# Sachin-A/TraceWeaver

Measured on AMD Instinct MI355X. Metric: spans/sec reconstructed + assignment accuracy vs ground truth, higher is better.
Workload: dtype int64 timestamps, f64 scores; 1 GPU; media_microservices shape (6 services, E in {1,1,1,1,2,4}), 100000 requests/service x 16 replicas per GPU, concurrency 1.6, two-pass reconstruction, device mixture refit; spans_per_gpu=25600000, spans_total=25600000, parallelism=units sharded, 1 rank(s), backend none

## Files before the change

traceweaver_amd/csrc/tw_engine.hip:

```cpp
#include <algorithm>
#include <chrono>
#include <cmath>
#include <cstdio>
#include <cstdlib>
#include <cstring>
#include <functional>
#include <string>
#include <type_traits>
#include <utility>
#include <vector>

#include <hip/hip_runtime.h>
#include <rocprim/rocprim.hpp>

#include "traceweaver_amd.h"
#include "tw_kernels.h"
#include "tw_fit.h"
#include "tw_eval.h"
#include "tw_skip.h"
#include "tw_load.h"
#include "tw_baselines.h"
#include "tw_stitch.h"
#include "tw_attr.h"
#include "tw_conf.h"
// ... 24 lines not shown
struct Knobs {
    int tile;
    int tile_threads;
    int tile_single;
    int tile_single_threads;
    int tile_pair;
    int tile_pair_threads;
    int tile_rank;
    int block_params;
    int coop;
    int set_hw_queues;
    int pipeline;
    int sig_hash_bits;
    int debug_lists;
    int stage_min_tiles;
    int tile_sub;
    int lean_pool;
    int split_twins, defer_min_e, lean_min_e, lean_grid, tile_max_deep;
    int64_t part_slots_max;
    int part_budget_deep;
    int fit_sort;
    int stage_gate;
    int fit_spec;
    int fit_order;
};

Knobs read_knobs() {
    Knobs K;
    K.tile = std::min(std::max(env_int("TW_TILE", kTile), 1), kTile);
    K.tile_threads = std::min(std::max(env_int("TW_TILE_THREADS", 2), 1), 4);
    K.tile_single = env_int("TW_TILE_SINGLE", 1);
    K.tile_single_threads = std::min(std::max(env_int("TW_TILE_SINGLE_THREADS", 1), 1), 4);
    K.tile_pair = env_int("TW_TILE_PAIR", 1);
    K.tile_pair_threads = std::min(std::max(env_int("TW_TILE_PAIR_THREADS", 2), 1), 2);
    K.tile_rank = env_int("TW_TILE_RANK", 1) != 0 ? 1 : 0;
    K.block_params = env_int("TW_BLOCK_PARAMS", 1);
    K.coop = std::min(std::max(env_int("TW_COOP_THREADS", kCoop), 1), kCoop);
    K.set_hw_queues = env_int("TW_SET_HW_QUEUES", 0);
    K.pipeline = env_int("TW_CLASS_PIPELINE", 1);
    K.sig_hash_bits = std::min(std::max(env_int("TW_SIG_HASH_BITS", 64), 1), 64);
    K.debug_lists = env_int("TW_DEBUG_LISTS", 0);
    K.stage_min_tiles = env_int("TW_STAGE_MIN_TILES", 1024);
    K.tile_sub = std::max(env_int("TW_TILE_SUB", 8), 1);
    K.lean_pool = std::min(std::max(env_int("TW_LEAN_POOL", 512), 1), 4096);
    K.split_twins = env_int("TW_SPLIT_TWINS", 2);
    K.defer_min_e = env_int("TW_DEFER_MIN_E", 5);
    K.lean_min_e = env_int("TW_LEAN_MIN_E", 5);
    K.lean_grid = std::max(env_int("TW_LEAN_GRID", TW_LEAN_GRID), 1);
    K.tile_max_deep = std::min(std::max(env_int("TW_TILE_MAX_DEEP", kTileMax), 0), kTileMax);
    K.part_slots_max = (int64_t)std::max(env_int("TW_PART_SLOTS_MAX", 16 << 20), 1024);
    K.part_budget_deep = env_int("TW_PART_BUDGET_DEEP", 2);
    K.fit_sort = env_int("TW_FIT_SORT", 0);
    K.stage_gate = env_int("TW_STAGE_GATE", 1);
    K.fit_spec = env_int("TW_FIT_SPEC", 1) != 0 ? 1 : 0;
    K.fit_order = env_int("TW_FIT_ORDER", 1) != 0 ? 1 : 0;
    return K;
}

struct Mt19937 {
    uint32_t mt[624];
    int idx = 624;
    explicit Mt19937(uint32_t seed = 0u) {
        mt[0] = seed;
        for (int i = 1; i < 624; i++) mt[i] = 1812433253u * (mt[i - 1] ^ (mt[i - 1] >> 30)) + (uint32_t)i;
    }
    uint32_t next() {
        if (idx >= 624) {
            for (int i = 0; i < 624; i++) {
                const uint32_t y = (mt[i] & 0x80000000u) | (mt[(i + 1) % 624] & 0x7fffffffu);
                mt[i] = mt[(i + 397) % 624] ^ (y >> 1) ^ ((y & 1u) ? 0x9908b0dfu : 0u);
            }
            idx = 0;
        }
        uint32_t y = mt[idx++];
        y ^= y >> 11;
        y ^= (y << 7) & 0x9d2c5680u;
        y ^= (y << 15) & 0xefc60000u;
        y ^= y >> 18;
// ... 40 lines not shown
    void* sort_tmp = nullptr;
    size_t sort_tmp_bytes = 0;
    double* mix_p_dev = nullptr;
    int32_t* mix_n_dev = nullptr;
    double* mix_c_dev = nullptr;
    double* gaps_sorted = nullptr;
    double* fit_models = nullptr;
    double* fit_uval = nullptr;
    int32_t *fit_ustart = nullptr, *fit_row_n = nullptr, *fit_row_uniq = nullptr;
    double* fit_centres = nullptr;
    hipEvent_t fit_fork = nullptr, fit_join = nullptr;
    double *fit_spec_centres = nullptr, *fit_spec_p = nullptr;
    int32_t *fit_spec_failed = nullptr, *fit_spec_ctr = nullptr;
    int32_t fit_spec_count[2] = {0, 0};
    double *fit_tape = nullptr, *fit_tape100 = nullptr;
    int64_t* fit_tape_off = nullptr;
    int64_t fit_tape_cap = 0;
    bool fit_runs_pending = false;
    bool fit_prepared = false;
    int32_t hard_pass1[kMaxEp + 1] = {};
    int8_t wide_pass1[kMaxEp + 1] = {};
    int32_t split_pass1[kMaxEp + 1] = {};
    bool pass1_done = false;
    std::vector<int32_t> fit_rows_h;
    bool fit_rows_h_valid = false;
    std::vector<int32_t> fit_order_h;
    int32_t* fit_order_dev = nullptr;
    double fit_order_host_ms = 0.0;
    Mt19937 fit_rng;
    uint32_t fit_seed = 0;
    int32_t* slot_unit = nullptr;
    int32_t* tile_ids = nullptr;
    int32_t* ctr = nullptr;
    int64_t ctr_round_ints = 0, ctr_pass_ints = 0;
    int32_t tile_cls_off[kMaxEp + 2] = {};
    BlockRef* blk_tab = nullptr;
    int32_t blk_cls_off[kMaxEp + 2] = {};
    uint32_t *seg_gap = nullptr, *seg_gap_end = nullptr, *seg_gap_dst = nullptr;
    unsigned long long *comp_a = nullptr, *comp_b = nullptr;
    int64_t comp_cap = 0, n_gap_scored = 0;
    int32_t *truth = nullptr, *in_trace = nullptr;
    uint8_t* trace_bad = nullptr;
    unsigned long long* eval_counts = nullptr;
    int64_t n_traces = 0, trace_cap = 0;
    uint8_t* slot_scored = nullptr;
    int64_t n_gap_rows = 0;
    unsigned long long* key_acc = nullptr;
    double fit_ms = 0.0;
    int rounds = 0;
    bool skip_mode = false;
// ... 226 lines not shown
        if (side.values) (void)hipFree(side.values);
        if (side.off) (void)hipFree(side.off);
        if (side.count) (void)hipFree(side.count);
        if (side.sum) (void)hipFree(side.sum);
        side = tw_engine::HistSide{};
    }
    void* rest[] = {e->hist_tile_off, e->hist_inv, e->hist_counters, e->hist_src_off, e->hist_src_values, e->hist_src_count, e->hist_src_sum};
    for (void* q : rest)
        if (q) (void)hipFree(q);
    e->hist_tile_off = nullptr; e->hist_inv = nullptr; e->hist_counters = nullptr; e->hist_plan_cap = 0; e->hist_inv_cap = 0;
    e->hist_src_off = e->hist_src_values = nullptr; e->hist_src_count = e->hist_src_sum = nullptr; e->hist_src_seg_cap = 0; e->hist_src_cap = 0;
    e->hist_cur = 0; e->hist_C = 0; e->hist_G = 0; e->hist_items = 0; e->hist_pushes = 0;
}

void chist_free(tw_engine* e) {
    ChistDev& H = e->CH;
    void* all[] = {H.table, H.off, H.entries, H.hash, H.stamp, H.cls, H.cell, H.src_hash, H.src_id, H.new_src, H.chunk_sum, H.counters, e->ch_up};
    for (void* q : all)
        if (q) (void)hipFree(q);
    H = ChistDev{};
    e->ch_mode = 0; e->ch_G = 0; e->ch_pushes = 0; e->ch_src_cap = 0; e->ch_up = nullptr; e->ch_up_bytes = 0;
}

void free_all(tw_engine* e) {
    for (void* q : e->allocs) (void)hipFree(q);
    e->allocs.clear();
    e->orig_is = e->orig_ie = e->orig_os = e->orig_oe = nullptr; e->orig_truth = e->orig_trace = nullptr;
    e->truth = nullptr; e->in_trace = nullptr; e->trace_bad = nullptr; e->eval_counts = nullptr; e->n_traces = 0; e->trace_cap = 0;
    drop_buffers(e);
    e->state = ST_EMPTY;
}

const char* kernel_error_text(int code) {
    switch (code) {
        case TW_ERR_WINDOW_WIDTH: return "an incoming span has more candidate spans at one endpoint than the candidate bitmap holds";
        case TW_ERR_WINDOW_SIZE: return "a window holds more than TW_MAX_WINDOW incoming spans";
        case TW_ERR_NAN_PARAMS: return "a parameter block holds a single sample (std = NaN); the reference aborts here (n_in % 100 == 1)";
        case TW_ERR_SKIP_PARAMS: return "skip mode: the scorer needs a (mean, std) pair that BuildDistributions did not produce (the reference raises KeyError)";
        case TW_ERR_SKIP_REFERENCE_RAISES: return "skip mode: the reference raises on this input (all endpoints skipped, or a score tie compared through a skip span)";
        case TW_ERR_ARG: return "skip mode: a request starts before the first time window";
        default: return "kernel reported an error";
    }
}

template <class Tr>
int run_scan(tw_engine* e, const TileSet& S, hipStream_t st, typename Tr::T* agg) {
    const Dev& P = e->P;
    hipLaunchKernelGGL((k_scan_local<Tr>), dim3(S.n), dim3(e->K.tile), 0, st, P, S, agg);
    hipLaunchKernelGGL((k_scan_spine<Tr>), dim3(P.n_units), dim3(e->K.coop), 0, st, P, S, agg);
// ... 846 lines not shown
            D.part_used = c + o_pu; D.split_count = c + o_sc; D.err = c + o_err; D.unit_ndirty = c + o_nd;
            D.redo_count = c + o_rd; D.fb_count = c + o_fc; D.defer_refused = c + o_dr; D.fb_total = c + o_ft; D.pair_busy = c + o_pb; D.any_wide = c + o_aw;
            D.unit_stats = (int64_t*)(c + o_us);
        };
        if (e->arena_open) e->arena_req.emplace_back(place, ((size_t)at * sizeof(int32_t) + 255) / 256 * 256);
        else { DEV_ALLOC(e->ctr, at); place(e->ctr); }
    }
    DEV_ALLOC(P.heavy_unit, sel_cap); DEV_ALLOC(P.heavy_win, sel_cap);
    DEV_ALLOC(P.tiny_unit, sel_cap); DEV_ALLOC(P.tiny_win, sel_cap);
    DEV_ALLOC(P.rheavy_unit, sel_cap); DEV_ALLOC(P.rheavy_win, sel_cap); DEV_ALLOC(P.rtiny_unit, sel_cap); DEV_ALLOC(P.rtiny_win, sel_cap);
    DEV_ALLOC(P.hard_unit, sel_cap / (kBruteMax + 1) + 1 + kSelSlots); DEV_ALLOC(P.hard_win, sel_cap / (kBruteMax + 1) + 1 + kSelSlots);
    DEV_ALLOC(e->rank_in, n_in_total); DEV_ALLOC(e->rank_out, n_out_total);
    DEV_ALLOC(e->agg_pair, P.n_tiles); DEV_ALLOC(e->agg_i32, P.n_tiles); DEV_ALLOC(e->agg_i32b, P.n_tiles);
    DEV_ALLOC(e->seg_in, (int64_t)seg_in.size()); DEV_ALLOC(e->seg_out, (int64_t)seg_out.size());
    DEV_ALLOC(e->gaps_sorted, gaps); DEV_ALLOC(e->fit_models, slots * kMaxComp * kModelStride);
    DEV_ALLOC(e->fit_uval, gaps); DEV_ALLOC(e->fit_ustart, gaps); DEV_ALLOC(e->fit_row_n, 2 * slots + 1);
    DEV_ALLOC(e->fit_tape, slots * kFitRowTape); DEV_ALLOC(e->fit_tape_off, slots); DEV_ALLOC(e->fit_tape100, kMaxComp * 13);
    e->fit_tape_cap = slots * kFitRowTape;
    DEV_ALLOC(e->fit_centres, slots * kMaxComp * (kMaxComp + 1));
    DEV_ALLOC(e->fit_spec_centres, slots * (kMaxComp + 1)); DEV_ALLOC(e->fit_spec_p, slots * kMaxComp * 3);
    DEV_ALLOC(e->fit_spec_failed, slots); DEV_ALLOC(e->fit_spec_ctr, 2);
    DEV_ALLOC(e->fit_order_dev, slots * (2 * kMaxComp));
    e->fit_order_h.clear();
    DEV_ALLOC(e->slot_unit, slots); DEV_ALLOC(e->slot_scored, slots);
    DEV_ALLOC(e->seg_gap, (int64_t)seg_gap_h.size()); DEV_ALLOC(e->seg_gap_end, (int64_t)seg_gap_end_h.size()); DEV_ALLOC(e->seg_gap_dst, (int64_t)seg_gap_dst_h.size());
    e->comp_cap = std::max(std::max(n_in_total, n_out_total), e->n_gap_scored);
    DEV_ALLOC(e->comp_a, e->comp_cap); DEV_ALLOC(e->comp_b, e->comp_cap);
    e->skip_mode = b->skip != nullptr;
    std::vector<int32_t> perm_h, pool_h;
    std::vector<int64_t> tw_h;
    std::vector<double> dist_h;
    std::vector<SkipUnitDev> skip_h;
    std::vector<int64_t> sk_tw_off, sk_pool_off, sk_dist_off;
    if (e->skip_mode) {
        perm_h.resize((size_t)n_out_total);
        for (int u = 0; u < b->n_units; u++) {
            const UnitDev& U = e->units[(size_t)u];
            const tw_skip_unit& K = b->skip[u];
            for (int k = 0; k < U.E; k++) {
                const int64_t a = U.ep_off[k], m = U.ep_off[k + 1] - a;
                std::vector<int32_t> idx((size_t)m);
                for (int64_t q = 0; q < m; q++) idx[(size_t)q] = (int32_t)q;
                std::stable_sort(idx.begin(), idx.end(), [&](int32_t x, int32_t y) { return b->out_start[a + x] < b->out_start[a + y]; });
                std::copy(idx.begin(), idx.end(), perm_h.begin() + a);
            }
            sk_tw_off.push_back((int64_t)tw_h.size()); sk_pool_off.push_back((int64_t)pool_h.size()); sk_dist_off.push_back((int64_t)dist_h.size());
// ... 132 lines not shown

namespace {

FitDev fit_dev(tw_engine* e) {
    FitDev F{};
    F.units = e->P.units; F.n_units = e->P.n_units; F.n_slots = e->n_slots; F.gaps = e->P.gaps; F.sorted = e->gaps_sorted;
    F.gs_off = e->P.gs_off; F.slot_unit = e->slot_unit; F.slot_scored = e->slot_scored; F.models = e->fit_models; F.mix_n = e->mix_n_dev; F.mix_p = e->mix_p_dev;
    F.uval = e->fit_uval; F.ustart = e->fit_ustart; F.row_n = e->fit_row_n; F.row_uniq = e->fit_row_uniq;
    F.tape = e->fit_tape; F.tape_off = e->fit_tape_off; F.tape100 = e->fit_tape100; F.err = e->P.err; F.centres = e->fit_centres;
    F.full_mode = FIT_FINAL; F.spec_centres = e->fit_spec_centres; F.spec_p = e->fit_spec_p; F.spec_failed = e->fit_spec_failed; F.spec_ctr = e->fit_spec_ctr;
    return F;
}

int fit_prepare_launch(tw_engine* e) {
    e->fit_runs_pending = false;
    if (e->fit_prepared || e->K.fit_sort != 0) return TW_OK;
    int32_t* flag = e->fit_row_n + 2 * e->n_slots;
    HIPCHK(hipMemsetAsync(flag, 0, sizeof(int32_t), e->stream));
#ifdef TW_HOST_EMULATION
    const int runs_threads = e->K.coop;
#else
    const int runs_threads = e->K.coop >= 64 ? kRunsThreads : e->K.coop;
#endif
    hipLaunchKernelGGL(k_fit_runs, dim3((unsigned)e->n_slots), dim3(runs_threads), 0, e->stream, fit_dev(e), flag);
    HIPCHK(hipGetLastError());
    e->fit_runs_pending = true;
    return TW_OK;
}
int fit_rows_to_host(tw_engine* e) {
    e->fit_rows_h.resize((size_t)(2 * e->n_slots + 1));
    HIPCHK(hipMemcpyAsync(e->fit_rows_h.data(), e->fit_row_n, sizeof(int32_t) * e->fit_rows_h.size(), hipMemcpyDeviceToHost, e->stream));
    return TW_OK;
}
int fit_prepare(tw_engine* e) {
    if (e->fit_prepared) return TW_OK;
    if (e->K.fit_sort == 0) {
        if (!e->fit_runs_pending) { int rl = fit_prepare_launch(e); if (rl != TW_OK) return rl; }
        e->fit_runs_pending = false;
        TWCHK(fit_rows_to_host(e));
        HIPCHK(hipStreamSynchronize(e->stream));
        if (!e->fit_rows_h[(size_t)(2 * e->n_slots)]) {
            e->fit_prepared = true;
            e->fit_rows_h_valid = true;
            return TW_OK;
        }
    }
    const unsigned size = (unsigned)e->n_gaps, nseg = (unsigned)e->n_gap_rows;
    unsigned long long kb[2];
    int rck = key_bits(e, e->P.gaps, e->seg_gap, e->seg_gap_end, (int)nseg, e->n_gaps, kb);
    if (rck != TW_OK) return rck;
    unsigned begin_bit = 0;
    if (kb[1] != 0 && !(kb[1] >> 63)) while (!((kb[1] >> begin_bit) & 1)) begin_bit++;
    if (kb[1] >> 63) {
        TWCHK(rocprim_call(e, [&](void* tmp, size_t& bytes) {
            return rocprim::segmented_radix_sort_keys(tmp, bytes, (const double*)e->P.gaps, e->gaps_sorted, size, nseg, e->seg_gap, e->seg_gap_end, 0, 64, e->stream);
        }));
    } else {
        int rcs = sort_rows(e, (const unsigned long long*)e->P.gaps, (unsigned long long*)e->gaps_sorted, size, e->seg_gap, e->seg_gap_end,
                            e->seg_gap_dst, (int)nseg, e->n_gap_scored, begin_bit, 64, 0ull);
        if (rcs != TW_OK) return rcs;
    }
    FitDev F = fit_dev(e);
#ifdef TW_HOST_EMULATION
    const int compress_threads = e->K.coop;
#else
    const int compress_threads = e->K.coop >= 64 ? kCompressThreads : e->K.coop;
#endif
    hipLaunchKernelGGL(k_fit_compress, dim3((unsigned)e->n_slots), dim3(compress_threads), 0, e->stream, F);
    HIPCHK(hipGetLastError());
    TWCHK(fit_rows_to_host(e));
    HIPCHK(hipStreamSynchronize(e->stream));
    e->fit_prepared = true;
    e->fit_rows_h_valid = true;
    return TW_OK;
}

void fit_order(const int32_t* row_uniq, const int32_t* row_n, int64_t n_slots, std::vector<int32_t>& out) {
    out.resize((size_t)(n_slots * 2 * kMaxComp));
    std::vector<int32_t> rows;
    rows.reserve((size_t)n_slots);
    for (int64_t q = 0; q < n_slots; q++)
        if (row_n[q] > 0 && row_uniq[q] >= 1) rows.push_back((int32_t)q);
    std::stable_sort(rows.begin(), rows.end(), [&](int32_t a, int32_t b) { return row_uniq[a] > row_uniq[b]; });
    int64_t len[kMaxComp + 1];
    for (int k = 1; k <= kMaxComp; k++)
        len[k] = std::partition_point(rows.begin(), rows.end(), [&](int32_t q) { return row_uniq[q] >= k; }) - rows.begin();
    const auto merge = [&](int32_t* tab, int k_min) {
        int64_t at = 0, pos[kMaxComp + 1] = {};
        for (;;) {
            int best = 0;
            int64_t best_key = -1;
            for (int k = kMaxComp; k >= k_min; k--) {
                if (pos[k] >= len[k]) continue;
                const int64_t key = (int64_t)row_uniq[rows[(size_t)pos[k]]] * k;
                if (key > best_key) { best_key = key; best = k; }
            }
            if (best == 0) break;
            tab[at++] = (int32_t)((kMaxComp - best) * n_slots + rows[(size_t)pos[best]++]);
        }
        for (int k = kMaxComp; k >= k_min; k--)
            for (int64_t q = 0; q < n_slots; q++)
                if (!(row_n[q] > 0 && k <= row_uniq[q])) tab[at++] = (int32_t)((kMaxComp - k) * n_slots + q);
    };
    merge(out.data(), 2);
    merge(out.data() + n_slots * (kMaxComp - 1), 1);
    int32_t* tab = out.data() + n_slots * (2 * kMaxComp - 1);
    int64_t at = 0;
    for (const int32_t q : rows) tab[at++] = q;
    for (int64_t q = 0; q < n_slots; q++)
        if (!(row_n[q] > 0 && row_uniq[q] >= 1)) tab[at++] = (int32_t)q;
}

int fit_run(tw_engine* e) {
    static const std::vector<double> tape100 = [] {
        std::vector<double> t((size_t)kMaxComp * 13, 0.0);
        for (int k = 1; k <= kMaxComp; k++) {
            Mt19937 r(100u);
            for (int j = 0; j < fit_draws(k); j++) t[(size_t)(k - 1) * 13 + j] = r.random_sample();
        }
        return t;
    }();
    HIPCHK(hipMemcpyAsync(e->fit_tape100, tape100.data(), sizeof(double) * tape100.size(), hipMemcpyHostToDevice, e->stream));
    HIPCHK(hipMemsetAsync(e->P.err, 0, sizeof(int32_t), e->stream));
    FitDev F = fit_dev(e);
    const int threads = e->K.coop >= 64 ? kFitThreads : e->K.coop;
    const int32_t *order_seed = nullptr, *order_em = nullptr, *order_row = nullptr;
    e->fit_order_h.clear();
    e->fit_order_host_ms = 0.0;
    if (e->K.fit_order != 0) {
        if (!e->fit_rows_h_valid) return fail(e, TW_ERR_STATE, "refit: the rows' counts are not on the host (fit_prepare leaves them there)");
        const auto h0 = std::chrono::steady_clock::now();
        fit_order(e->fit_rows_h.data() + e->n_slots, e->fit_rows_h.data(), e->n_slots, e->fit_order_h);
        HIPCHK(hipMemcpyAsync(e->fit_order_dev, e->fit_order_h.data(), sizeof(int32_t) * e->fit_order_h.size(), hipMemcpyHostToDevice, e->stream));
        e->fit_order_host_ms = std::chrono::duration<double, std::milli>(std::chrono::steady_clock::now() - h0).count();
        order_seed = e->fit_order_dev;
        order_em = order_seed + e->n_slots * (kMaxComp - 1);
        order_row = order_em + e->n_slots * kMaxComp;
    }
    int side_cls = 0;
    for (int E = kMaxEp; E >= 1; E--)
        if (e->tile_cls_off[E + 1] > e->tile_cls_off[E]) side_cls = E;
    const hipStream_t side = e->cls_stream[side_cls];
    const bool spec = e->K.fit_spec != 0 && side_cls > 0;
    e->fit_spec_count[0] = e->fit_spec_count[1] = 0;
    if (spec) {
        HIPCHK(hipMemsetAsync(e->fit_spec_ctr, 0, 2 * sizeof(int32_t), e->stream));
        HIPCHK(hipEventRecord(e->fit_fork, e->stream));
        HIPCHK(hipStreamWaitEvent(side, e->fit_fork, 0));
        FitDev S = F;
        S.full_mode = FIT_SPEC;
        S.order = order_row;
        hipLaunchKernelGGL(k_fit_seed<true>, dim3((unsigned)e->n_slots), dim3(threads), 0, side, S);
        hipLaunchKernelGGL(k_fit_em<true>, dim3((unsigned)e->n_slots), dim3(threads), 0, side, S);
        HIPCHK(hipEventRecord(e->fit_join, side));
    }
    F.order = order_seed;
    hipLaunchKernelGGL(k_fit_seed<false>, dim3((unsigned)(e->n_slots * (kMaxComp - 1))), dim3(threads), 0, e->stream, F);
    F.order = order_em;
    hipLaunchKernelGGL(k_fit_em<false>, dim3((unsigned)(e->n_slots * kMaxComp)), dim3(threads), 0, e->stream, F);
    F.order = order_row;
    hipLaunchKernelGGL(k_fit_select, dim3((unsigned)((e->n_slots + 63) / 64)), dim3(64), 0, e->stream, F);
    if (spec) {
        HIPCHK(hipStreamWaitEvent(e->stream, e->fit_join, 0));
        F.full_mode = FIT_ADOPT;
    }
    hipLaunchKernelGGL(k_fit_seed<true>, dim3((unsigned)e->n_slots), dim3(threads), 0, e->stream, F);
    hipLaunchKernelGGL(k_fit_em<true>, dim3((unsigned)e->n_slots), dim3(threads), 0, e->stream, F);
    const int64_t total = e->n_slots * kMaxComp;
    hipLaunchKernelGGL(k_mix_consts, dim3((unsigned)((total + 255) / 256)), dim3(256), 0, e->stream, (const double*)e->mix_p_dev, (const int32_t*)e->mix_n_dev, (const int32_t*)e->slot_unit, e->P.units, e->mix_c_dev, total);
    HIPCHK(hipEventRecord(e->ev[EV_END], e->stream));
    HIPCHK(hipGetLastError());
    int32_t kerr = 0;
    HIPCHK(hipMemcpyAsync(&kerr, e->P.err, sizeof(int32_t), hipMemcpyDeviceToHost, e->stream));
    if (spec) HIPCHK(hipMemcpyAsync(e->fit_spec_count, e->fit_spec_ctr, 2 * sizeof(int32_t), hipMemcpyDeviceToHost, e->stream));
    HIPCHK(hipStreamSynchronize(e->stream));
    float f = 0.f;
    HIPCHK(hipEventElapsedTime(&f, e->ev[EV_BEGIN], e->ev[EV_END]));
    e->fit_ms = f;
    if (kerr != 0)
        return fail(e, kerr, "refit: every model-selection fit of an edge ended in a covariance <= 0 (scikit-learn's ValueError); the reference "
                             "raises there as well (np.argmin of an empty list, traceweaver_v3.py:777-780)");
    e->state = ST_MIX;
    return TW_OK;
}

int fit_check_state(tw_engine* e, const char* who) {
    if (e->state != ST_PASS1) return fail(e, TW_ERR_STATE, std::string(who) + " is valid right after tw_run_pass1");
    if (e->skip_mode) return fail(e, TW_ERR_STATE, "a skip-mode batch runs one pass (traceweaver_v3.py:1155-1156): there is no refit");
    return TW_OK;
}

}

int tw_set_fit_seed(tw_engine* e, uint32_t seed) {
// ... 12 lines not shown
    if (rc != TW_OK) return rc;
    for (int64_t q = 0; q < e->n_slots; q++) max_n[q] = std::min<int32_t>(e->fit_rows_h[(size_t)(e->n_slots + q)], kMaxComp);
    return TW_OK;
}

int tw_get_fit_order(tw_engine* e, int32_t* order_seed, int32_t* order_em, int32_t* order_row, int32_t* present) {
    if (e == nullptr || order_seed == nullptr || order_em == nullptr || order_row == nullptr || present == nullptr) return TW_ERR_ARG;
    if (e->state < ST_MIX) return fail(e, TW_ERR_STATE, "tw_get_fit_order: no refit has run on the resident batch");
    *present = e->fit_order_h.empty() ? 0 : 1;
    if (*present) {
        const size_t ns = (size_t)e->n_slots, k = (size_t)kMaxComp;
        std::copy_n(e->fit_order_h.data(), ns * (k - 1), order_seed);
        std::copy_n(e->fit_order_h.data() + ns * (k - 1), ns * k, order_em);
        std::copy_n(e->fit_order_h.data() + ns * (2 * k - 1), ns, order_row);
    }
    return TW_OK;
}

int tw_fit_mixtures_tape(tw_engine* e, const double* tape, int64_t tape_len, const int64_t* slot_off) {
    if (e == nullptr || tape == nullptr || slot_off == nullptr || tape_len < 0) return TW_ERR_ARG;
    int rc = fit_check_state(e, "tw_fit_mixtures_tape");
    if (rc != TW_OK) return rc;
    HIPCHK(hipSetDevice(e->device));
    rc = fit_prepare(e);
    if (rc != TW_OK) return rc;
    static const int need[kMaxComp + 1] = {0, 1, 4, 11, 21, 34};
    for (int64_t q = 0; q < e->n_slots; q++) {
        const int m = std::min<int32_t>(e->fit_rows_h[(size_t)(e->n_slots + q)], kMaxComp);
        if (m > 0 && (slot_off[q] < 0 || slot_off[q] + need[m] > tape_len))
            return fail(e, TW_ERR_ARG, "tw_fit_mixtures_tape: the tape does not hold the draws of slot " + std::to_string(q));
    }
    HIPCHK(hipEventRecord(e->ev[EV_BEGIN], e->stream));
    if (tape_len > e->fit_tape_cap) {
        double* p = nullptr;
        rc = dev_alloc(e, &p, tape_len);
        if (rc != TW_OK) return rc;
        e->fit_tape = p;
        e->fit_tape_cap = tape_len;
    }
    HIPCHK(hipMemcpyAsync(e->fit_tape, tape, sizeof(double) * (size_t)std::max<int64_t>(tape_len, 0), hipMemcpyHostToDevice, e->stream));
    HIPCHK(hipMemcpyAsync(e->fit_tape_off, slot_off, sizeof(int64_t) * e->n_slots, hipMemcpyHostToDevice, e->stream));
    return fit_run(e);
}

int tw_fit_mixtures_seeded(tw_engine* e, const uint32_t* unit_seed) {
    if (e == nullptr) return TW_ERR_ARG;
    int rc = fit_check_state(e, "tw_fit_mixtures");
    if (rc != TW_OK) return rc;
    HIPCHK(hipSetDevice(e->device));
    HIPCHK(hipEventRecord(e->ev[EV_BEGIN], e->stream));
    rc = fit_prepare_launch(e);
    if (rc != TW_OK) return rc;
    static thread_local std::vector<double> tape;
    static thread_local std::vector<int64_t> off;
    tape.resize((size_t)e->n_slots * kFitRowTape);
    off.resize((size_t)e->n_slots);
    for (int64_t q = 0; q < e->n_slots; q++) off[(size_t)q] = q * kFitRowTape;
    if (unit_seed == nullptr) {
        for (size_t i = 0; i < tape.size(); i++) tape[i] = e->fit_rng.random_sample();
    } else {
        for (size_t u = 0; u < e->units.size(); u++) {
            Mt19937 r(unit_seed[u]);
            const size_t lo = (size_t)e->units[u].slot_off * kFitRowTape, hi = lo + (size_t)e->units[u].nslot * kFitRowTape;
            for (size_t i = lo; i < hi; i++) tape[i] = r.random_sample();
        }
    }
    if ((int64_t)tape.size() > e->fit_tape_cap) return fail(e, TW_ERR_STATE, "tw_fit_mixtures: tape buffer smaller than the batch");
    HIPCHK(hipMemcpyAsync(e->fit_tape, tape.data(), sizeof(double) * tape.size(), hipMemcpyHostToDevice, e->stream));
    HIPCHK(hipMemcpyAsync(e->fit_tape_off, off.data(), sizeof(int64_t) * off.size(), hipMemcpyHostToDevice, e->stream));
    if (e->fit_prepared) HIPCHK(hipStreamSynchronize(e->stream));
    rc = fit_prepare(e);
    if (rc != TW_OK) return rc;
    return fit_run(e);
}

int tw_fit_mixtures(tw_engine* e) { return tw_fit_mixtures_seeded(e, nullptr); }

int tw_get_mixtures(tw_engine* e, int32_t* mix_n, double* mix_p) {
    if (e == nullptr || mix_n == nullptr || mix_p == nullptr) return TW_ERR_ARG;
    if (e->state < ST_MIX) return fail(e, TW_ERR_STATE, "no mixtures resident (tw_fit_mixtures / tw_set_mixtures first)");
    HIPCHK(hipSetDevice(e->device));
    HIPCHK(hipMemcpyAsync(mix_n, e->mix_n_dev, sizeof(int32_t) * e->n_slots, hipMemcpyDeviceToHost, e->stream));
    HIPCHK(hipMemcpyAsync(mix_p, e->mix_p_dev, sizeof(double) * e->n_slots * kMaxComp * 3, hipMemcpyDeviceToHost, e->stream));
    HIPCHK(hipStreamSynchronize(e->stream));
    return TW_OK;
}

int tw_run_pass2(tw_engine* e) {
    if (e == nullptr) return TW_ERR_ARG;
    if (e->state != ST_MIX && e->state != ST_PASS2) return fail(e, TW_ERR_STATE, "tw_run_pass2 needs tw_run_pass1 and tw_set_mixtures first");
    if (!e->pass1_done) return fail(e, TW_ERR_STATE, "tw_run_pass2 on a batch whose first pass has not run (tw_run_pass1 first)");
    HIPCHK(hipSetDevice(e->device));
// ... 34 lines not shown
    for (const UnitDev& U : e->units)
        for (int64_t q = U.gp_off; q < U.gp_off + (int64_t)U.nblk * U.nslot; q++) gauss[q * 3] *= U.tscale;
    return TW_OK;
}

int tw_get_timing(tw_engine* e, double* ms, int32_t n) {
    if (e == nullptr || ms == nullptr) return TW_ERR_ARG;
    for (int i = 0; i < n && i < 6; i++) ms[i] = e->ms[i];
    if (n > 6) ms[6] = e->fit_ms;
    if (n > 7) ms[7] = (double)e->rounds;
    if (n > 8) ms[8] = e->host_ms[0];
    if (n > 9) ms[9] = e->host_ms[1];
    for (int i = 0; i < 6 && 10 + i < n; i++) ms[10 + i] = e->st_ms[i];
    for (int i = 0; i < 3 && 16 + i < n; i++) ms[16 + i] = e->at_ms[i];
    for (int i = 0; i < 3 && 19 + i < n; i++) ms[19 + i] = e->cf_ms[i];
    for (int i = 0; i < 3 && 22 + i < n; i++) ms[22 + i] = e->ds_ms[i];
    for (int i = 0; i < 3 && 25 + i < n; i++) ms[25 + i] = e->sg_ms[i];
    for (int i = 0; i < 3 && 28 + i < n; i++) ms[28 + i] = e->pf_ms[i];
    if (n > 31) ms[31] = e->ob_ms;
    if (n > 32) ms[32] = (double)e->gate_waits;
    for (int i = 0; i < 2 && 33 + i < n; i++) ms[33 + i] = e->cm_ms[i];
    for (int i = 0; i < 2 && 35 + i < n; i++) ms[35 + i] = (double)e->fit_spec_count[i];
    if (n > 37) ms[37] = e->fit_order_host_ms;
    for (int i = 0; i < 3 && 43 + i < n; i++) ms[43 + i] = e->ch_ms[i];
    for (int i = 0; i < 3 && 46 + i < n; i++) ms[46 + i] = e->fl_ms[i];
    for (int i = 0; i < 3 && 49 + i < n; i++) ms[49 + i] = e->ex_ms[i];
    for (int i = 0; i < 5 && 38 + i < n; i++) ms[38 + i] = e->hs_ms[i];
    return TW_OK;
}

int tw_debug_profile_hist(tw_engine* e, unsigned long long* out16) {
    if (e == nullptr || out16 == nullptr || e->state < ST_LOADED) return TW_ERR_ARG;
    HIPCHK(hipMemcpyAsync(out16, e->P.prof + 16, sizeof(unsigned long long) * 16, hipMemcpyDeviceToHost, e->stream));
    HIPCHK(hipStreamSynchronize(e->stream));
    return TW_OK;
}

int tw_debug_profile(tw_engine* e, unsigned long long* out16) {
    if (e == nullptr || out16 == nullptr || e->state < ST_LOADED) return TW_ERR_ARG;
    HIPCHK(hipMemcpyAsync(out16, e->P.prof, sizeof(unsigned long long) * 16, hipMemcpyDeviceToHost, e->stream));
    HIPCHK(hipStreamSynchronize(e->stream));
    return TW_OK;
}

int tw_find_order(tw_engine* e, int32_t n_units, const int64_t* unit_in_off, const int32_t* unit_E, const int64_t* ep_off,
                  const int64_t* out_start, const int64_t* out_end, const int32_t* true_child, uint8_t* dag_out) {
// ... 2258 lines not shown
```

traceweaver_amd/csrc/tw_fit.h:

```cpp
#pragma once
#include "tw_device.h"

namespace tw {

#ifndef TW_FIT_THREADS
#define TW_FIT_THREADS 512
#endif
constexpr int kFitThreads = TW_FIT_THREADS;
constexpr int kFitWaves = kFitThreads / 64;
constexpr int kFitStats = 3 * kMaxComp + 2;
constexpr int kFitMaxIter = 100;
constexpr double kFitTol = 1.0e-3;
constexpr double kFitRegCovar = 1.0e-6;
constexpr int kKmMaxIter = 300;
constexpr double kKmTol = 1.0e-4;
constexpr double kEps10 = 10.0 * 2.220446049250313e-16;
constexpr int kModelStride = 1 + 3 * kMaxComp;
constexpr int kFitMaxTrials = 3;
constexpr int kFitRowTape = 34;

__host__ __device__ inline int fit_trials(int k) { return k < 3 ? 2 : 3; }
__host__ __device__ inline int fit_draws(int k) { return 1 + (k - 1) * fit_trials(k); }
__host__ __device__ inline int fit_tape_pos(int k) { return k == 1 ? 0 : k == 2 ? 1 : k == 3 ? 4 : k == 4 ? 11 : 21; }

// ... 100 lines not shown
            for (int w = 0; w < nwave; w++) { const int c = wave_heads[j][w]; if (w < wave) mine += c; chunk += c; }
            if (head[j]) {
                F.uval[row + pos + mine + before[j]] = xi[j];
                F.ustart[row + pos + mine + before[j]] = base + j * nt + t;
            }
            pos += chunk;
        }
        __syncthreads();
        if (t == 0) carry_sh = pos;
    }
    __syncthreads();
    if (t == 0) { F.row_n[q] = n_sh; F.row_uniq[q] = carry_sh; }
}

#ifndef TW_FIT_HASH_SLOTS
#define TW_FIT_HASH_SLOTS 16384
#endif
constexpr int kHashSlots = TW_FIT_HASH_SLOTS;
constexpr int kHashMax = kHashSlots / 4 * 3;
constexpr unsigned long long kHashEmpty = ~0ull;
constexpr int kRunsThreads = 1024;
static_assert((kHashSlots & (kHashSlots - 1)) == 0 && kHashSlots >= 64, "the table size is a power of two");

__global__ void __launch_bounds__(kRunsThreads) k_fit_runs(FitDev F, int32_t* fallback) {
    constexpr int R = 8;
    __shared__ unsigned long long tab[kHashSlots];
    __shared__ int32_t s_part[kRunsThreads / 64];
    __shared__ int32_t s_uniq, s_n, s_bad;
    const int64_t q = blockIdx.x;
    const int t = threadIdx.x, nt = blockDim.x;
    const int lane = t & 63, wave = t >> 6;
    if (!F.slot_scored[q]) {
        if (t == 0) { F.row_n[q] = 0; F.row_uniq[q] = 0; }
        return;
    }
    const UnitDev& U = F.units[F.slot_unit[q]];
    const int n_all = U.n_in;
    const int64_t row = F.gs_off[F.slot_unit[q]] + (q - U.slot_off) * (int64_t)n_all;
    const double* x = F.gaps + row;
    const double scale = U.tscale, inv = 1.0 / U.tscale;
    int slots = kHashSlots < 256 ? kHashSlots : 256;
    while (slots < kHashSlots && slots < 2 * n_all) slots <<= 1;
    const int slot_shift = 32 - __builtin_ctz((unsigned)slots), hash_max = slots / 4 * 3;
    for (int r = t; r < slots; r += nt) tab[r] = kHashEmpty;
    if (t == 0) { s_uniq = 0; s_n = 0; s_bad = 0; }
    __syncthreads();
    int mine = 0;
// ... 7 lines not shown
            mine++;
            const double v = xi[j] * inv;
            const uint32_t key = (uint32_t)v;
            if (__double_as_longlong(xi[j]) < 0 || !(v < 4294967295.0) || (double)key != v) { s_bad = 1; continue; }
            uint32_t slot = (key * 2654435761u) >> slot_shift;
            const unsigned long long word = (unsigned long long)key << 32;
            bool placed = false;
            for (int probe = 0; probe < slots && !placed; probe++) {
                const unsigned long long old = atomicCAS(&tab[slot], kHashEmpty, word);
                if (old == kHashEmpty) { if (atomicAdd(&s_uniq, 1) >= hash_max) s_bad = 1; placed = true; }
                else if ((uint32_t)(old >> 32) == key) placed = true;
                else slot = (slot + 1) & (uint32_t)(slots - 1);
            }
            if (placed) atomicAdd(&tab[slot], 1ull); else s_bad = 1;
        }
        if (s_bad) break;
    }
    atomicAdd(&s_n, mine);
    __syncthreads();
    if (s_bad) {
        if (t == 0) atomicExch(fallback, 1);
        return;
    }
    for (int k = 2; k <= slots; k <<= 1) {
        for (int j = k >> 1; j >= 1; j >>= 1) {
            for (int p = t; p < slots / 2; p += nt) {
                const int i = ((p & ~(j - 1)) << 1) | (p & (j - 1));
                const unsigned long long a = tab[i], b = tab[i | j];
                const bool up = (i & k) == 0;
                if ((a > b) == up) { tab[i] = b; tab[i | j] = a; }
            }
            __syncthreads();
        }
    }
    const int uniq = s_uniq, per = (uniq + nt - 1) / nt;
    const int r_lo = t * per < uniq ? t * per : uniq, r_hi = r_lo + per < uniq ? r_lo + per : uniq;
    int sum = 0;
    for (int r = r_lo; r < r_hi; r++) sum += (int)(uint32_t)tab[r];
    int inc = sum;
    for (int off = 1; off < 64; off <<= 1) { const int o = __shfl_up(inc, off); if (lane >= off) inc += o; }
    if (lane == 63 || t == nt - 1) s_part[wave] = inc;
    __syncthreads();
    int before = inc - sum;
    for (int w = 0; w < wave; w++) before += s_part[w];
    for (int r = r_lo; r < r_hi; r++) {
        const unsigned long long w = tab[r];
        F.uval[row + r] = (double)(uint32_t)(w >> 32) * scale;
        F.ustart[row + r] = before;
        before += (int)(uint32_t)w;
    }
    if (t == 0) { F.row_n[q] = s_n; F.row_uniq[q] = uniq; }
}

__device__ __forceinline__ double fit_dist(double c, double x) {
    double d = -2.0 * (c * x);
    d += c * c;
    d += x * x;
    return d > 0.0 ? d : 0.0;
// ... 563 lines not shown
```

traceweaver_amd/engine.py:

```python
import ctypes
import os
import warnings

import numpy as np

from . import _ffi


class EngineError(RuntimeError):
    def __init__(self, code, message):
        super().__init__("%s (%d): %s" % (_ffi.STATUS.get(code, "TW_ERR"), code, message))
        self.code = code


class UnitArrays(object):

    AFTER_CUT, BEFORE_CUT = 1, 2

    def __init__(self, in_start, in_end, out_off, out_start, out_end, dag, key_rank=None, time_scale=None, part=0):
        self.time_scale = None if time_scale is None else float(time_scale)
        self.part = int(part)
        self.in_start = np.ascontiguousarray(in_start, dtype=np.int64)
        self.in_end = np.ascontiguousarray(in_end, dtype=np.int64)
        self.out_off = np.ascontiguousarray(out_off, dtype=np.int64)
# ... 846 lines not shown
        val = np.empty(len(start), dtype=np.int64)
        self._check(self._lib.tw_build_distributions(self._h, len(start), _vp(start), _vp(dur), _vp(ep), int(large_delay), int(E), _vp(key), _vp(val)))
        return key, val

    def hbm_copy_gbps(self, nbytes=1 << 30, iters=10):
        g = ctypes.c_double(0.0)
        self._check(self._lib.tw_measure_hbm_copy(self._h, int(nbytes), int(iters), ctypes.byref(g)))
        return float(g.value)

    def timing(self):
        ms = np.zeros(10, dtype=np.float64)
        self._check(self._lib.tw_get_timing(self._h, _vp(ms), 10))
        return dict(zip(("pass", "enumerate", "select", "windows", "repair", "params", "fit", "rounds", "host_enum_submit", "host_pass"), ms.tolist()))

    def gated_stages(self):
        ms = np.zeros(33, dtype=np.float64)
        self._check(self._lib.tw_get_timing(self._h, _vp(ms), 33))
        return int(ms[32])

    def fit_spec(self):
        ms = np.zeros(37, dtype=np.float64)
        self._check(self._lib.tw_get_timing(self._h, _vp(ms), 37))
        return int(ms[35]), int(ms[36])
```

Before: 1.556 billion spans/s.

## Compact hash table before bitonic sort and pin refit staging buffers

In k_fit_runs, occupied hash slots are now compacted to the front of the shared table with a block-wide prefix scan. The bitonic sort then runs only over the next power of two above the unique count, not the full table. The refit's host tape, offsets, order tables and row counts move into one page-locked block so their async copies can be real DMA. The constant tape100 upload and the memsets are queued earlier, before the prepare sync. This adds a compaction pass and extra timing bookkeeping, and the host order tables are copied back into the vector after launch.

```diff
diff --git a/traceweaver_amd/csrc/tw_engine.hip b/traceweaver_amd/csrc/tw_engine.hip
--- a/traceweaver_amd/csrc/tw_engine.hip
+++ b/traceweaver_amd/csrc/tw_engine.hip
@@ -70,6 +70,8 @@
     int fit_sort;
     int stage_gate;
     int fit_spec;
+    int fit_runs_compact;
+    int fit_head;
     int fit_order;
 };
 
@@ -102,6 +104,8 @@
     K.stage_gate = env_int("TW_STAGE_GATE", 1);
     K.fit_spec = env_int("TW_FIT_SPEC", 1) != 0 ? 1 : 0;
     K.fit_order = env_int("TW_FIT_ORDER", 1) != 0 ? 1 : 0;
+    K.fit_runs_compact = env_int("TW_FIT_RUNS_COMPACT", 1) != 0 ? 1 : 0;
+    K.fit_head = env_int("TW_FIT_HEAD", 1) != 0 ? 1 : 0;
     return K;
 }
 
@@ -188,10 +192,20 @@
     int8_t wide_pass1[kMaxEp + 1] = {};
     int32_t split_pass1[kMaxEp + 1] = {};
     bool pass1_done = false;
-    std::vector<int32_t> fit_rows_h;
+    void* fit_pin = nullptr;
+    double *fit_pin_tape = nullptr, *fit_pin_tape100 = nullptr;
+    int64_t* fit_pin_off = nullptr;
+    int32_t *fit_pin_order = nullptr;
+    int fit_sort_route = 0;
+    bool fit_head_queued = false;
+    bool fit_wait_end_valid = false;
+    std::chrono::steady_clock::time_point fit_wait_end;
+    std::vector<int32_t> fit_rows_vec;
+    int32_t* fit_rows_h = nullptr;
     bool fit_rows_h_valid = false;
     std::vector<int32_t> fit_order_h;
     int32_t* fit_order_dev = nullptr;
+    double fit_launch_host_ms = 0.0;
     double fit_order_host_ms = 0.0;
     Mt19937 fit_rng;
     uint32_t fit_seed = 0;
@@ -464,9 +478,24 @@
     e->ch_mode = 0; e->ch_G = 0; e->ch_pushes = 0; e->ch_src_cap = 0; e->ch_up = nullptr; e->ch_up_bytes = 0;
 }
 
+const std::vector<double>& fit_tape100() {
+    static const std::vector<double> tape100 = [] {
+        std::vector<double> t((size_t)kMaxComp * 13, 0.0);
+        for (int k = 1; k <= kMaxComp; k++) {
+            Mt19937 r(100u);
+            for (int j = 0; j < fit_draws(k); j++) t[(size_t)(k - 1) * 13 + j] = r.random_sample();
+        }
+        return t;
+    }();
+    return tape100;
+}
+
 void free_all(tw_engine* e) {
     for (void* q : e->allocs) (void)hipFree(q);
     e->allocs.clear();
+    if (e->fit_pin != nullptr) (void)hipHostFree(e->fit_pin);
+    e->fit_pin = nullptr; e->fit_pin_tape = e->fit_pin_tape100 = nullptr; e->fit_pin_off = nullptr; e->fit_pin_order = nullptr; e->fit_rows_h = nullptr;
+    e->fit_head_queued = false; e->fit_wait_end_valid = false;
     e->orig_is = e->orig_ie = e->orig_os = e->orig_oe = nullptr; e->orig_truth = e->orig_trace = nullptr;
     e->truth = nullptr; e->in_trace = nullptr; e->trace_bad = nullptr; e->eval_counts = nullptr; e->n_traces = 0; e->trace_cap = 0;
     drop_buffers(e);
@@ -1359,6 +1388,20 @@
     DEV_ALLOC(e->fit_spec_failed, slots); DEV_ALLOC(e->fit_spec_ctr, 2);
     DEV_ALLOC(e->fit_order_dev, slots * (2 * kMaxComp));
     e->fit_order_h.clear();
+    if (e->K.fit_head != 0) {
+        const size_t n_tape = (size_t)slots * kFitRowTape, n_100 = (size_t)kMaxComp * 13, n_order = (size_t)slots * 2 * kMaxComp, n_rows = (size_t)(2 * slots + 1);
+        const size_t bytes = sizeof(double) * (n_tape + n_100) + sizeof(int64_t) * (size_t)slots + sizeof(int32_t) * (n_order + n_rows);
+        if (hipHostMalloc(&e->fit_pin, std::max<size_t>(bytes, 8), hipHostMallocDefault) != hipSuccess) { e->fit_pin = nullptr; return fail(e, TW_ERR_DEVICE, "tw_load_batch: out of page-locked host memory (the refit's staging block)"); }
+        e->fit_pin_tape = (double*)e->fit_pin; e->fit_pin_tape100 = e->fit_pin_tape + n_tape;
+        e->fit_pin_off = (int64_t*)(e->fit_pin_tape100 + n_100);
+        e->fit_pin_order = (int32_t*)(e->fit_pin_off + slots);
+        e->fit_rows_h = e->fit_pin_order + n_order;
+        const std::vector<double>& t100 = fit_tape100();
+        std::copy(t100.begin(), t100.end(), e->fit_pin_tape100);
+    } else {
+        e->fit_rows_vec.assign((size_t)(2 * slots + 1), 0);
+        e->fit_rows_h = e->fit_rows_vec.data();
+    }
     DEV_ALLOC(e->slot_unit, slots); DEV_ALLOC(e->slot_scored, slots);
     DEV_ALLOC(e->seg_gap, (int64_t)seg_gap_h.size()); DEV_ALLOC(e->seg_gap_end, (int64_t)seg_gap_end_h.size()); DEV_ALLOC(e->seg_gap_dst, (int64_t)seg_gap_dst_h.size());
     e->comp_cap = std::max(std::max(n_in_total, n_out_total), e->n_gap_scored);
@@ -1537,14 +1580,13 @@
 #else
     const int runs_threads = e->K.coop >= 64 ? kRunsThreads : e->K.coop;
 #endif
-    hipLaunchKernelGGL(k_fit_runs, dim3((unsigned)e->n_slots), dim3(runs_threads), 0, e->stream, fit_dev(e), flag);
+    hipLaunchKernelGGL(k_fit_runs, dim3((unsigned)e->n_slots), dim3(runs_threads), 0, e->stream, fit_dev(e), flag, e->K.fit_runs_compact);
     HIPCHK(hipGetLastError());
     e->fit_runs_pending = true;
     return TW_OK;
 }
 int fit_rows_to_host(tw_engine* e) {
-    e->fit_rows_h.resize((size_t)(2 * e->n_slots + 1));
-    HIPCHK(hipMemcpyAsync(e->fit_rows_h.data(), e->fit_row_n, sizeof(int32_t) * e->fit_rows_h.size(), hipMemcpyDeviceToHost, e->stream));
+    HIPCHK(hipMemcpyAsync(e->fit_rows_h, e->fit_row_n, sizeof(int32_t) * (size_t)(2 * e->n_slots + 1), hipMemcpyDeviceToHost, e->stream));
     return TW_OK;
 }
 int fit_prepare(tw_engine* e) {
@@ -1554,7 +1596,9 @@
         e->fit_runs_pending = false;
         TWCHK(fit_rows_to_host(e));
         HIPCHK(hipStreamSynchronize(e->stream));
+        e->fit_wait_end = std::chrono::steady_clock::now(); e->fit_wait_end_valid = true;
         if (!e->fit_rows_h[(size_t)(2 * e->n_slots)]) {
+            e->fit_sort_route = 0;
             e->fit_prepared = true;
             e->fit_rows_h_valid = true;
             return TW_OK;
@@ -1585,13 +1629,14 @@
     HIPCHK(hipGetLastError());
     TWCHK(fit_rows_to_host(e));
     HIPCHK(hipStreamSynchronize(e->stream));
+    e->fit_wait_end = std::chrono::steady_clock::now(); e->fit_wait_end_valid = true;
+    e->fit_sort_route = 1;
     e->fit_prepared = true;
     e->fit_rows_h_valid = true;
     return TW_OK;
 }
 
-void fit_order(const int32_t* row_uniq, const int32_t* row_n, int64_t n_slots, std::vector<int32_t>& out) {
-    out.resize((size_t)(n_slots * 2 * kMaxComp));
+void fit_order(const int32_t* row_uniq, const int32_t* row_n, int64_t n_slots, int32_t* out) {
     std::vector<int32_t> rows;
     rows.reserve((size_t)n_slots);
     for (int64_t q = 0; q < n_slots; q++)
@@ -1617,26 +1662,29 @@
             for (int64_t q = 0; q < n_slots; q++)
                 if (!(row_n[q] > 0 && k <= row_uniq[q])) tab[at++] = (int32_t)((kMaxComp - k) * n_slots + q);
     };
-    merge(out.data(), 2);
-    merge(out.data() + n_slots * (kMaxComp - 1), 1);
-    int32_t* tab = out.data() + n_slots * (2 * kMaxComp - 1);
+    merge(out, 2);
+    merge(out + n_slots * (kMaxComp - 1), 1);
+    int32_t* tab = out + n_slots * (2 * kMaxComp - 1);
     int64_t at = 0;
     for (const int32_t q : rows) tab[at++] = q;
     for (int64_t q = 0; q < n_slots; q++)
         if (!(row_n[q] > 0 && row_uniq[q] >= 1)) tab[at++] = (int32_t)q;
 }
 
+int fit_head_queue(tw_engine* e) {
+    const double* t100 = e->fit_pin_tape100 != nullptr ? e->fit_pin_tape100 : fit_tape100().data();
+    HIPCHK(hipMemcpyAsync(e->fit_tape100, t100, sizeof(double) * (size_t)kMaxComp * 13, hipMemcpyHostToDevice, e->stream));
+    HIPCHK(hipMemsetAsync(e->P.err, 0, sizeof(int32_t), e->stream));
+    HIPCHK(hipMemsetAsync(e->fit_spec_ctr, 0, 2 * sizeof(int32_t), e->stream));
+    e->fit_head_queued = true;
+    return TW_OK;
+}
+
 int fit_run(tw_engine* e) {
-    static const std::vector<double> tape100 = [] {
-        std::vector<double> t((size_t)kMaxComp * 13, 0.0);
-        for (int k = 1; k <= kMaxComp; k++) {
-            Mt19937 r(100u);
-            for (int j = 0; j < fit_draws(k); j++) t[(size_t)(k - 1) * 13 + j] = r.random_sample();
-        }
-        return t;
-    }();
-    HIPCHK(hipMemcpyAsync(e->fit_tape100, tape100.data(), sizeof(double) * tape100.size(), hipMemcpyHostToDevice, e->stream));
-    HIPCHK(hipMemsetAsync(e->P.err, 0, sizeof(int32_t), e->stream));
+    const auto wait_end = e->fit_wait_end_valid ? e->fit_wait_end : std::chrono::steady_clock::now();
+    e->fit_wait_end_valid = false;
+    if (!e->fit_head_queued) TWCHK(fit_head_queue(e));
+    e->fit_head_queued = false;
     FitDev F = fit_dev(e);
     const int threads = e->K.coop >= 64 ? kFitThreads : e->K.coop;
     const int32_t *order_seed = nullptr, *order_em = nullptr, *order_row = nullptr;
@@ -1645,8 +1693,11 @@
     if (e->K.fit_order != 0) {
         if (!e->fit_rows_h_valid) return fail(e, TW_ERR_STATE, "refit: the rows' counts are not on the host (fit_prepare leaves them there)");
         const auto h0 = std::chrono::steady_clock::now();
-        fit_order(e->fit_rows_h.data() + e->n_slots, e->fit_rows_h.data(), e->n_slots, e->fit_order_h);
-        HIPCHK(hipMemcpyAsync(e->fit_order_dev, e->fit_order_h.data(), sizeof(int32_t) * e->fit_order_h.size(), hipMemcpyHostToDevice, e->stream));
+        const size_t n_order = (size_t)(e->n_slots * 2 * kMaxComp);
+        if (e->fit_pin_order == nullptr) e->fit_order_h.resize(n_order);
+        int32_t* tables = e->fit_pin_order != nullptr ? e->fit_pin_order : e->fit_order_h.data();
+        fit_order(e->fit_rows_h + e->n_slots, e->fit_rows_h, e->n_slots, tables);
+        HIPCHK(hipMemcpyAsync(e->fit_order_dev, tables, sizeof(int32_t) * n_order, hipMemcpyHostToDevice, e->stream));
         e->fit_order_host_ms = std::chrono::duration<double, std::milli>(std::chrono::steady_clock::now() - h0).count();
         order_seed = e->fit_order_dev;
         order_em = order_seed + e->n_slots * (kMaxComp - 1);
@@ -1659,7 +1710,6 @@
     const bool spec = e->K.fit_spec != 0 && side_cls > 0;
     e->fit_spec_count[0] = e->fit_spec_count[1] = 0;
     if (spec) {
-        HIPCHK(hipMemsetAsync(e->fit_spec_ctr, 0, 2 * sizeof(int32_t), e->stream));
         HIPCHK(hipEventRecord(e->fit_fork, e->stream));
         HIPCHK(hipStreamWaitEvent(side, e->fit_fork, 0));
         FitDev S = F;
@@ -1685,6 +1735,9 @@
     hipLaunchKernelGGL(k_mix_consts, dim3((unsigned)((total + 255) / 256)), dim3(256), 0, e->stream, (const double*)e->mix_p_dev, (const int32_t*)e->mix_n_dev, (const int32_t*)e->slot_unit, e->P.units, e->mix_c_dev, total);
     HIPCHK(hipEventRecord(e->ev[EV_END], e->stream));
     HIPCHK(hipGetLastError());
+    e->fit_launch_host_ms = std::chrono::duration<double, std::milli>(std::chrono::steady_clock::now() - wait_end).count();
+    if (e->fit_pin_order != nullptr && e->K.fit_order != 0)
+        e->fit_order_h.assign(e->fit_pin_order, e->fit_pin_order + (size_t)(e->n_slots * 2 * kMaxComp));
     int32_t kerr = 0;
     HIPCHK(hipMemcpyAsync(&kerr, e->P.err, sizeof(int32_t), hipMemcpyDeviceToHost, e->stream));
     if (spec) HIPCHK(hipMemcpyAsync(e->fit_spec_count, e->fit_spec_ctr, 2 * sizeof(int32_t), hipMemcpyDeviceToHost, e->stream));
@@ -1743,6 +1796,7 @@
     int rc = fit_check_state(e, "tw_fit_mixtures_tape");
     if (rc != TW_OK) return rc;
     HIPCHK(hipSetDevice(e->device));
+    e->fit_head_queued = false;
     rc = fit_prepare(e);
     if (rc != TW_OK) return rc;
     static const int need[kMaxComp + 1] = {0, 1, 4, 11, 21, 34};
@@ -1769,16 +1823,19 @@
     int rc = fit_check_state(e, "tw_fit_mixtures");
     if (rc != TW_OK) return rc;
     HIPCHK(hipSetDevice(e->device));
+    e->fit_head_queued = false;
     HIPCHK(hipEventRecord(e->ev[EV_BEGIN], e->stream));
     rc = fit_prepare_launch(e);
     if (rc != TW_OK) return rc;
-    static thread_local std::vector<double> tape;
-    static thread_local std::vector<int64_t> off;
-    tape.resize((size_t)e->n_slots * kFitRowTape);
-    off.resize((size_t)e->n_slots);
+    static thread_local std::vector<double> tape_vec;
+    static thread_local std::vector<int64_t> off_vec;
+    const size_t n_tape = (size_t)e->n_slots * kFitRowTape, n_off = (size_t)e->n_slots;
+    if (e->fit_pin == nullptr) { tape_vec.resize(n_tape); off_vec.resize(n_off); }
+    double* tape = e->fit_pin != nullptr ? e->fit_pin_tape : tape_vec.data();
+    int64_t* off = e->fit_pin != nullptr ? e->fit_pin_off : off_vec.data();
     for (int64_t q = 0; q < e->n_slots; q++) off[(size_t)q] = q * kFitRowTape;
     if (unit_seed == nullptr) {
-        for (size_t i = 0; i < tape.size(); i++) tape[i] = e->fit_rng.random_sample();
+        for (size_t i = 0; i < n_tape; i++) tape[i] = e->fit_rng.random_sample();
     } else {
         for (size_t u = 0; u < e->units.size(); u++) {
             Mt19937 r(unit_seed[u]);
@@ -1786,9 +1843,10 @@
             for (size_t i = lo; i < hi; i++) tape[i] = r.random_sample();
         }
     }
-    if ((int64_t)tape.size() > e->fit_tape_cap) return fail(e, TW_ERR_STATE, "tw_fit_mixtures: tape buffer smaller than the batch");
-    HIPCHK(hipMemcpyAsync(e->fit_tape, tape.data(), sizeof(double) * tape.size(), hipMemcpyHostToDevice, e->stream));
-    HIPCHK(hipMemcpyAsync(e->fit_tape_off, off.data(), sizeof(int64_t) * off.size(), hipMemcpyHostToDevice, e->stream));
+    if ((int64_t)n_tape > e->fit_tape_cap) return fail(e, TW_ERR_STATE, "tw_fit_mixtures: tape buffer smaller than the batch");
+    HIPCHK(hipMemcpyAsync(e->fit_tape, tape, sizeof(double) * n_tape, hipMemcpyHostToDevice, e->stream));
+    HIPCHK(hipMemcpyAsync(e->fit_tape_off, off, sizeof(int64_t) * n_off, hipMemcpyHostToDevice, e->stream));
+    if (e->K.fit_head != 0) TWCHK(fit_head_queue(e));
     if (e->fit_prepared) HIPCHK(hipStreamSynchronize(e->stream));
     rc = fit_prepare(e);
     if (rc != TW_OK) return rc;
@@ -1869,6 +1927,8 @@
     for (int i = 0; i < 2 && 33 + i < n; i++) ms[33 + i] = e->cm_ms[i];
     for (int i = 0; i < 2 && 35 + i < n; i++) ms[35 + i] = (double)e->fit_spec_count[i];
     if (n > 37) ms[37] = e->fit_order_host_ms;
+    if (n > 52) ms[52] = e->fit_launch_host_ms;
+    if (n > 53) ms[53] = (double)e->fit_sort_route;
     for (int i = 0; i < 3 && 43 + i < n; i++) ms[43 + i] = e->ch_ms[i];
     for (int i = 0; i < 3 && 46 + i < n; i++) ms[46 + i] = e->fl_ms[i];
     for (int i = 0; i < 3 && 49 + i < n; i++) ms[49 + i] = e->ex_ms[i];
diff --git a/traceweaver_amd/csrc/tw_fit.h b/traceweaver_amd/csrc/tw_fit.h
--- a/traceweaver_amd/csrc/tw_fit.h
+++ b/traceweaver_amd/csrc/tw_fit.h
@@ -146,7 +146,7 @@
 constexpr int kRunsThreads = 1024;
 static_assert((kHashSlots & (kHashSlots - 1)) == 0 && kHashSlots >= 64, "the table size is a power of two");
 
-__global__ void __launch_bounds__(kRunsThreads) k_fit_runs(FitDev F, int32_t* fallback) {
+__global__ void __launch_bounds__(kRunsThreads) k_fit_runs(FitDev F, int32_t* fallback, int compact) {
     constexpr int R = 8;
     __shared__ unsigned long long tab[kHashSlots];
     __shared__ int32_t s_part[kRunsThreads / 64];
@@ -200,9 +200,42 @@
         if (t == 0) atomicExch(fallback, 1);
         return;
     }
-    for (int k = 2; k <= slots; k <<= 1) {
+    const int uniq = s_uniq;
+    if (compact != 0) {
+        constexpr int C = 16;
+        const int nwave = (nt + 63) >> 6;
+        int base = 0;
+        for (int r0 = 0; r0 < slots; r0 += nt * C) {
+            unsigned long long w[C];
+            int cnt = 0;
+#pragma unroll
+            for (int c = 0; c < C; c++) {
+                const int r = r0 + t * C + c;
+                w[c] = r < slots ? tab[r] : kHashEmpty;
+                cnt += w[c] != kHashEmpty;
+            }
+            int inc = cnt;
+            for (int off = 1; off < 64; off <<= 1) { const int o = __shfl_up(inc, off); if (lane >= off) inc += o; }
+            if (lane == 63 || t == nt - 1) s_part[wave] = inc;
+            __syncthreads();
+            int at = base + inc - cnt;
+            for (int wv = 0; wv < nwave; wv++) { const int s = s_part[wv]; if (wv < wave) at += s; base += s; }
+#pragma unroll
+            for (int c = 0; c < C; c++)
+                if (w[c] != kHashEmpty) tab[at++] = w[c];
+            __syncthreads();
+        }
+    }
+    int sorted = slots;
+    if (compact != 0) {
+        sorted = 64 < slots ? 64 : slots;
+        while (sorted < uniq) sorted <<= 1;
+        for (int r = uniq + t; r < sorted; r += nt) tab[r] = kHashEmpty;
+        __syncthreads();
+    }
+    for (int k = 2; k <= sorted; k <<= 1) {
         for (int j = k >> 1; j >= 1; j >>= 1) {
-            for (int p = t; p < slots / 2; p += nt) {
+            for (int p = t; p < sorted / 2; p += nt) {
                 const int i = ((p & ~(j - 1)) << 1) | (p & (j - 1));
                 const unsigned long long a = tab[i], b = tab[i | j];
                 const bool up = (i & k) == 0;
@@ -211,7 +244,7 @@
             __syncthreads();
         }
     }
-    const int uniq = s_uniq, per = (uniq + nt - 1) / nt;
+    const int per = (uniq + nt - 1) / nt;
     const int r_lo = t * per < uniq ? t * per : uniq, r_hi = r_lo + per < uniq ? r_lo + per : uniq;
     int sum = 0;
     for (int r = r_lo; r < r_hi; r++) sum += (int)(uint32_t)tab[r];
diff --git a/traceweaver_amd/engine.py b/traceweaver_amd/engine.py
--- a/traceweaver_amd/engine.py
+++ b/traceweaver_amd/engine.py
@@ -892,3 +892,8 @@
         ms = np.zeros(37, dtype=np.float64)
         self._check(self._lib.tw_get_timing(self._h, _vp(ms), 37))
         return int(ms[35]), int(ms[36])
+
+    def fit_head(self):
+        ms = np.zeros(54, dtype=np.float64)
+        self._check(self._lib.tw_get_timing(self._h, _vp(ms), 54))
+        return {"order_ms": float(ms[37]), "launch_ms": float(ms[52]), "sort_route": bool(ms[53])}
```

Result: no change. 1.568 billion spans/s (median of 6 runs) (+0.8%).
